# hanmekim/SceneLib2

Hardware: AMD Instinct MI355X
Metric: batched MonoSLAM frames/sec (320x240, 100 feat) (higher is better)
Workload: dtype f64

## Files before the change

scenelib2_amd/csrc/sl2_frontend.hip:

```cpp
#include "sl2_frontend_dev.hpp"

namespace sl2 {

__global__ void __launch_bounds__(256) k_predict(double* __restrict__ x, double* __restrict__ P, const int* __restrict__ n_slots,
                                                 double* __restrict__ prev_r, const int* __restrict__ part_i, int pend, int ld,
                                                 double* __restrict__ seq_time, const uint8_t* __restrict__ active) {
  if (!active[blockIdx.x]) { predict_paused(blockIdx.x, seq_time); return; }
  predict_body(blockIdx.x, x, P, n_slots, prev_r, part_i, pend, ld, seq_time);
}

__global__ void __launch_bounds__(64) k_feature_prediction(const double* __restrict__ x, const double* __restrict__ P,
                                                           const double* __restrict__ xp_org, int* __restrict__ f_flags,
                                                           const int* __restrict__ n_slots, double* __restrict__ f_h,
                                                           double* __restrict__ f_Hx, double* __restrict__ f_Hy,
                                                           double* __restrict__ f_R, double* __restrict__ f_S,
                                                           double* __restrict__ f_score, int* __restrict__ srch_i, double* __restrict__ srch_d,
                                                           const double* __restrict__ seq_cam, int width, int height, int N, int ld,
                                                           const uint8_t* __restrict__ active) {
  if (!active[blockIdx.y]) return;
  const CameraParams cam = load_cam(seq_cam, blockIdx.y, width, height);
  feature_prediction_body(blockIdx.y, blockIdx.x * blockDim.x + threadIdx.x, x, P, xp_org, f_flags, n_slots, f_h, f_Hx, f_Hy, f_R, f_S,
                          f_score, srch_i, srch_d, cam, N, ld);
}

__global__ void __launch_bounds__(256) k_select(const double* __restrict__ f_score, int* __restrict__ f_flags,
                                                const int* __restrict__ n_slots, const double* __restrict__ xp_org,
                                                int* __restrict__ sel_idx, int* __restrict__ n_sel, int* __restrict__ n_vis,
                                                double* __restrict__ last_r, const int* __restrict__ srch_i,
                                                const double* __restrict__ srch_d, int* __restrict__ srch_sel, int N,
                                                int n_want, int* __restrict__ srch_big, int split_bands,
                                                const uint8_t* __restrict__ active, int* __restrict__ sel_gate) {
  extern __shared__ double s_dyn[];
  if (!active[blockIdx.x]) { select_paused(blockIdx.x, sel_gate); return; }
  select_body(blockIdx.x, f_score, f_flags, n_slots, xp_org, sel_idx, n_sel, n_vis, last_r, srch_i, srch_d, srch_sel, N, n_want,
              srch_big, split_bands, s_dyn, sel_gate);
}

__global__ void __launch_bounds__(128) k_finalize(double* __restrict__ x, double* __restrict__ P, int* __restrict__ f_flags,
                                                  const int* __restrict__ n_slots, int* __restrict__ attempted,
                                                  int* __restrict__ successful, const int* __restrict__ m_count,
                                                  const int* __restrict__ n_sel, double* __restrict__ traj,
                                                  int* __restrict__ traj_count, const double* __restrict__ last_r,
                                                  int* __restrict__ status, double* __restrict__ pos_log, int* __restrict__ pos_count, int N, int ld,
                                                  int min_attempts, double match_fraction, int save_trajectory,
                                                  const int* __restrict__ part_i, int pend, int* __restrict__ slots_max,
                                                  unsigned long long* __restrict__ slots_mail, int publish,
                                                  const uint8_t* __restrict__ active, int* __restrict__ seq_age) {
  extern __shared__ int s_del[];
  if (!active[blockIdx.x]) { finalize_paused(blockIdx.x, x, n_slots, pos_log, pos_count, seq_age, ld, slots_max, slots_mail, publish); return; }
  finalize_body(blockIdx.x, x, P, f_flags, n_slots, attempted, successful, m_count, n_sel, traj, traj_count, last_r, status, pos_log,
                pos_count, N, ld, min_attempts, match_fraction, save_trajectory, part_i, pend, s_del, slots_max, slots_mail, publish);
}

#ifdef SL2_FRONT_TRACE
}
extern "C" int sl2_debug_front_trace(long long* dev_buf) {
  return hipMemcpyToSymbol(HIP_SYMBOL(sl2::g_front_trace), &dev_buf, sizeof(dev_buf)) == hipSuccess ? 0 : 2;
}
namespace sl2 {
#endif

int launch_predict(sl2_engine* e) {
  LaunchScope ls(e, "k_predict");
  hipLaunchKernelGGL(k_predict, dim3(e->B), dim3(256), 0, e->stream, e->x, e->P, e->n_slots, e->prev_r, e->part_i, e->ppos + 6 * e->kpart, e->ld,
                     e->seq_time, e->active);
  SL2_HIP(hipGetLastError());
  return SL2_OK;
}

int launch_feature_prediction(sl2_engine* e) {
  LaunchScope ls(e, "k_feature_prediction");
  dim3 grid((e->N + 63) / 64, e->B);
  hipLaunchKernelGGL(k_feature_prediction, grid, dim3(64), 0, e->stream, e->x, e->P, e->xp_org, e->f_flags, e->n_slots,
                     e->f_h, e->f_Hx, e->f_Hy, e->f_R, e->f_S, e->f_score, e->srch_i, e->srch_d, e->seq_cam, e->cam.width, e->cam.height, e->N, e->ld,
                     e->active);
  SL2_HIP(hipGetLastError());
  return SL2_OK;
}

int launch_select(sl2_engine* e, int n) {
  LaunchScope ls(e, "k_select");
  if (n > e->nsel_max) n = e->nsel_max;
  const size_t shm = (size_t)e->N * (sizeof(double) + 3 * sizeof(int));
  hipLaunchKernelGGL(k_select, dim3(e->B), dim3(256), shm, e->stream, e->f_score, e->f_flags, e->n_slots, e->xp_org,
                     e->sel_idx, e->n_sel, e->n_vis, e->last_r, e->srch_i, e->srch_d, e->srch_sel, e->N, n, e->srch_big,
                     (e->srch_big && e->root->search_variant == 1) ? e->root->search_split : 0, e->active, e->sel_gate);
  SL2_HIP(hipGetLastError());
  return SL2_OK;
}

int launch_finalize(sl2_engine* e, int save_trajectory) {
  LaunchScope ls(e, "k_finalize");
  const size_t shm = (size_t)e->N * 2 * sizeof(int);
  hipLaunchKernelGGL(k_finalize, dim3(e->B), dim3(128), shm, e->stream, e->x, e->P, e->f_flags, e->n_slots, e->attempted,
                     e->successful, e->m_count, e->n_sel, e->traj, e->traj_count, e->last_r, e->status, e->pos_log,
                     e->pos_count, e->N, e->ld, e->prm.minimum_attempted_measurements_of_feature,
                     e->prm.successful_match_fraction, save_trajectory, e->part_i, e->ppos + 6 * e->kpart, e->root->slots_max_dev,
                     e->root->slots_mail_dev, e->group_first == 0 ? 1 : 0, e->active, e->seq_age);
  SL2_HIP(hipGetLastError());
  return SL2_OK;
}

}
```

scenelib2_amd/csrc/sl2_frontend_dev.hpp:

```cpp
#pragma once
#include "sl2_common.hpp"

namespace sl2 {

#ifdef SL2_FRONT_TRACE
static __device__ long long* g_front_trace = nullptr;
#define FTR(kern, slot) do { if (g_front_trace && threadIdx.x == 0) g_front_trace[((size_t)(kern) * 4096 + blockIdx.x) * 8 + (slot)] = (long long)__builtin_readcyclecounter(); } while (0)
#else
#define FTR(kern, slot) do { } while (0)
#endif

__device__ __forceinline__ void predict_body(const int b, double* __restrict__ x, double* __restrict__ P, const int* __restrict__ n_slots,
                                                 double* __restrict__ prev_r, const int* __restrict__ part_i, int pend, int ld,
                                                 double* __restrict__ seq_time) {
  const int tid = threadIdx.x;
  double* xb = x + (size_t)b * ld;
  double* Pb = P + (size_t)b * ld * ld;
  FTR(0, 0);
  if (tid < 3) prev_r[b * 3 + tid] = xb[tid];
  const int n_used = part_i[(size_t)b * kPartInts + kPartCount] ? pend : 13 + 3 * n_slots[b];
  double v0[13];
  for (int k = 0; k < 13; ++k) v0[k] = (13 + tid < n_used) ? Pb[(size_t)k * ld + 13 + tid] : 0.0;
  __shared__ double s_f[13], s_A[16], s_B[12], s_P[169], s_T[169], s_dt;
  if (tid == 0) {
    double* rec = seq_time + (size_t)b * kSeqTimeDoubles;
    const double dt0 = rec[kSeqTimeNominal] + rec[kSeqTimeOwed];
    double xv[13];
    for (int i = 0; i < 13; ++i) xv[i] = xb[i];
    rec[kSeqTimeUsed] = dt0;
    rec[kSeqTimeOwed] = 0.0;
    s_dt = dt0;
    double f[13], A44[16], B43[12];
    motion_f_and_blocks(xv, dt0, f, A44, B43);
    for (int i = 0; i < 13; ++i) s_f[i] = f[i];
    for (int i = 0; i < 16; ++i) s_A[i] = A44[i];
    for (int i = 0; i < 12; ++i) s_B[i] = B43[i];
  }
  for (int e = tid; e < 169; e += blockDim.x) s_P[e] = Pb[(size_t)(e / 13) * ld + (e % 13)];
  __syncthreads();
  const double dt = s_dt;
  FTR(0, 1);
  for (int e = tid; e < 169; e += blockDim.x) {
    const int i = e / 13, j = e % 13;
    double v[13];
    for (int k = 0; k < 13; ++k) v[k] = s_P[k * 13 + j];
    s_T[e] = frow_dot(i, dt, s_A, s_B, v);
  }
  __syncthreads();
  FTR(0, 2);
  for (int e = tid; e < 169; e += blockDim.x) {
    const int i = e / 13, j = e % 13;
    double v[13];
    for (int k = 0; k < 13; ++k) v[k] = s_T[i * 13 + k];
    Pb[(size_t)i * ld + j] = frow_dot(j, dt, s_A, s_B, v) + process_noise_entry(i, j, dt, s_B);
  }
  FTR(0, 3);
  __shared__ double s_W[256][13];
  for (int j0 = 13; j0 < n_used; j0 += blockDim.x) {
    const int j = j0 + tid;
    if (j < n_used) {
      double v[13], w[13];
      for (int k = 0; k < 13; ++k) v[k] = (j0 == 13) ? v0[k] : Pb[(size_t)k * ld + j];
      for (int i = 0; i < 13; ++i) w[i] = frow_dot(i, dt, s_A, s_B, v);
      for (int i = 0; i < 13; ++i) {
        Pb[(size_t)i * ld + j] = w[i];
        s_W[tid][i] = w[i];
      }
    }
    __syncthreads();
    const int rr = tid >> 4, cc = tid & 15;
    for (int r0 = 0; r0 < (int)blockDim.x; r0 += blockDim.x / 16) {
      const int jr = j0 + r0 + rr;
      if (cc < 13 && jr < n_used) Pb[(size_t)jr * ld + cc] = s_W[r0 + rr][cc];
    }
    __syncthreads();
  }
  if (tid < 13) xb[tid] = s_f[tid];
  FTR(0, 4);
}

__device__ __forceinline__ void predict_paused(const int b, double* __restrict__ seq_time) {
  if (threadIdx.x == 0) {
    double* rec = seq_time + (size_t)b * kSeqTimeDoubles;
    if (rec[kSeqTimeCatchUp] != 0.0) rec[kSeqTimeOwed] += rec[kSeqTimeNominal];
  }
}

__device__ __forceinline__ void feature_prediction_body(const int b, const int i, const double* __restrict__ x, const double* __restrict__ P,
                                                           const double* __restrict__ xp_org, int* __restrict__ f_flags,
                                                           const int* __restrict__ n_slots, double* __restrict__ f_h,
                                                           double* __restrict__ f_Hx, double* __restrict__ f_Hy,
                                                           double* __restrict__ f_R, double* __restrict__ f_S,
                                                           double* __restrict__ f_score, int* __restrict__ srch_i, double* __restrict__ srch_d,
                                                           const CameraParams& cam, int N, int ld) {
  if (i >= n_slots[b]) return;
  const size_t fi = (size_t)b * N + i;
  int flags = f_flags[fi] & ~(FF_SELECTED | FF_VISIBLE);
  if (!(flags & FF_ACTIVE)) { f_flags[fi] = flags; return; }
  const double* xb = x + (size_t)b * ld;
  const double* Pb = P + (size_t)b * ld * ld;
  double xp[7], y[3], xo[7];
  for (int k = 0; k < 7; ++k) xp[k] = xb[k];
  const int pos = 13 + 3 * i;
  for (int k = 0; k < 3; ++k) y[k] = xb[pos + k];
  for (int k = 0; k < 7; ++k) xo[k] = xp_org[fi * 8 + k];
  double zeroed[3], h[2], Hx[14], Hy[6], Rn;
  measurement_model(cam, xp, y, zeroed, h, Hx, Hy, &Rn);
  double Pxx7[49], Pxy7[21], Pyy[9], S[4];
  for (int r = 0; r < 7; ++r) {
    for (int c = 0; c < 7; ++c) Pxx7[r * 7 + c] = Pb[(size_t)r * ld + c];
    for (int c = 0; c < 3; ++c) Pxy7[r * 3 + c] = Pb[(size_t)r * ld + pos + c];
  }
  for (int r = 0; r < 3; ++r)
    for (int c = 0; c < 3; ++c) Pyy[r * 3 + c] = Pb[(size_t)(pos + r) * ld + pos + c];
  innovation_cov(Hx, Hy, Rn, Pxx7, Pxy7, Pyy, S);
  const int cant_see = visibility_test(cam, xp, y, xo, h);
  f_h[fi * 2 + 0] = h[0]; f_h[fi * 2 + 1] = h[1];
  for (int k = 0; k < 14; ++k) f_Hx[fi * 14 + k] = Hx[k];
  for (int k = 0; k < 6; ++k) f_Hy[fi * 6 + k] = Hy[k];
  f_R[fi] = Rn;
  for (int k = 0; k < 4; ++k) f_S[fi * 4 + k] = S[k];
  f_score[fi] = S[0] + S[3];
  if (cant_see == 0) flags |= FF_VISIBLE;
  f_flags[fi] = flags;
  {
    double a, bq, c;
    sinv_from_S(S, &a, &bq, &c);
    const SearchBounds sb = search_bounds(h, a, bq, c, cam.width, cam.height);
    int* si = srch_i + fi * 8;
    si[0] = sb.ucentre; si[1] = sb.vcentre; si[2] = sb.urelstart; si[3] = sb.urelfinish - sb.urelstart + 1;
    si[4] = sb.vrelstart; si[5] = sb.vrelfinish - sb.vrelstart + 1; si[6] = sb.halfwidth; si[7] = sb.halfheight;
    double* sd = srch_d + fi * 4;
    sd[0] = a; sd[1] = bq; sd[2] = c; sd[3] = 0.0;
  }
}

__device__ __forceinline__ void select_body(const int b, const double* __restrict__ f_score, int* __restrict__ f_flags,
                                                const int* __restrict__ n_slots, const double* __restrict__ xp_org,
                                                int* __restrict__ sel_idx, int* __restrict__ n_sel, int* __restrict__ n_vis,
                                                double* __restrict__ last_r, const int* __restrict__ srch_i,
                                                const double* __restrict__ srch_d, int* __restrict__ srch_sel, int N,
                                                int n_want, int* __restrict__ srch_big, int split_bands, double* s_dyn,
                                                int* __restrict__ sel_gate) {
  double* s_score = s_dyn;
  int* s_vis = (int*)(s_dyn + N);
  int* s_nu = s_vis + N;
  __shared__ int s_nvis, s_zero_rank, s_last;
  const int tid = threadIdx.x;
  FTR(1, 0);
  const int ns = n_slots[b];
  if (tid == 0) { s_nvis = 0; s_zero_rank = 0x7fffffff; s_last = -1; }
  __syncthreads();
  for (int i0 = 0; i0 < ns; i0 += blockDim.x) {
    const int i = i0 + tid;
    int last = -1;
    if (i < ns) {
      const int fl = f_flags[(size_t)b * N + i];
      s_score[i] = f_score[(size_t)b * N + i];
      s_vis[i] = (fl & FF_VISIBLE) ? 1 : 0;
      if (fl & FF_ACTIVE) last = i;
    }
    for (int off = 32; off > 0; off >>= 1) last = max(last, __shfl_xor(last, off, 64));
    if ((tid & 63) == 0 && last >= 0) atomicMax(&s_last, last);
  }
  __syncthreads();
  FTR(1, 1);
  for (int i = tid; i < ns; i += blockDim.x) {
    if (!s_vis[i]) s_score[i] = -1.0;
    else if (s_score[i] != s_score[i]) s_score[i] = -0.5;
    s_nu[i] = 0;
  }
  __syncthreads();
  {
    const int G = (ns + 63) / 64 * 64;
    int P = G > 0 ? (int)blockDim.x / G : 1;
    P = P < 1 ? 1 : (P > 4 ? 4 : P);
    const int part = P > 1 ? tid / G : 0;
    for (int i = P > 1 ? tid - part * G : tid; i < ns && part < P; i += P > 1 ? ns : (int)blockDim.x) {
      if (!s_vis[i]) continue;
      const double si = s_score[i];
      const int j0 = part * ns / P, j1 = (part + 1) * ns / P;
      int rank = 0;
#pragma unroll 8
      for (int j = j0; j < j1; ++j) {
        const double sj = s_score[j];
        rank += (sj > si || (sj == si && j < i)) ? 1 : 0;
      }
      if (P > 1) atomicAdd(&s_nu[i], rank); else s_nu[i] = rank;
    }
  }
  __syncthreads();
  for (int i0 = 0; i0 < ns; i0 += blockDim.x) {
    const int i = i0 + tid;
    const bool vis = i < ns && s_vis[i];
    int zero_rank = 0x7fffffff;
    if (vis) {
      const int rank = s_nu[i];
      s_vis[i] = 1 + rank;
      if (s_score[i] == 0.0) zero_rank = rank;
    }
    const int nv = __popcll(__ballot(vis));
    for (int off = 32; off > 0; off >>= 1) zero_rank = min(zero_rank, __shfl_xor(zero_rank, off, 64));
    if ((tid & 63) == 0) {
      if (nv) atomicAdd(&s_nvis, nv);
      if (zero_rank != 0x7fffffff) atomicMin(&s_zero_rank, zero_rank);
    }
  }
  __syncthreads();
  FTR(1, 2);
  int limit = n_want;
  if (s_zero_rank < limit) limit = s_zero_rank;
  if (s_nvis < limit) limit = s_nvis;
  for (int i = tid; i < ns; i += blockDim.x) {
    if (!s_vis[i]) continue;
    const int rank = s_vis[i] - 1;
    if (rank < limit) {
      sel_idx[(size_t)b * N + rank] = i;
      f_flags[(size_t)b * N + i] |= FF_SELECTED;
      const int* si = srch_i + ((size_t)b * N + i) * 8;
      int* rec = srch_sel + ((size_t)b * N + rank) * 16;
      rec[0] = i;
#pragma unroll
      for (int q = 0; q < 7; ++q) rec[1 + q] = si[q];
      const double* sd = srch_d + ((size_t)b * N + i) * 4;
      double* recd = (double*)(rec + 8);
      recd[0] = sd[0]; recd[1] = sd[1]; recd[2] = sd[2];
      int shared = 0;
      if (split_bands > 0 && si[3] > 0 && si[5] > 0) {
        const int TU = (si[3] + 15) >> 4, TV = (si[5] + 15) >> 4;
        const int bands = ((TU + 1) >> 1) * TV;
        if (bands >= split_bands && TU <= 128 && TV <= 64) {
          const int per = srch_unit_bands(bands), units = (bands + per - 1) / per;
          const int u0 = atomicAdd(srch_big, units);
          if (u0 + units <= kSrchBigUnits) {
            int4 en;
            en.x = b; en.y = rank; en.z = u0; en.w = units;
            for (int q = 0; q < units; ++q) *(int4*)(srch_big + kSrchBigEntries + 4 * (u0 + q)) = en;
            atomicAdd(srch_big + 3, 1);
            shared = 1;
          } else {
            int4 en;
            en.x = -1; en.y = 0; en.z = 0; en.w = 0;
            for (int q = u0; q < min(u0 + units, kSrchBigUnits); ++q) *(int4*)(srch_big + kSrchBigEntries + 4 * q) = en;
          }
        }
      }
      rec[14] = shared ? si[3] : 0;
      if (shared) rec[4] = kSrchSharedNu;
    }
  }
  FTR(1, 3);
  if (tid == 0) {
    n_sel[b] = limit;
    sel_gate[b] = limit;
    n_vis[b] = s_nvis;
    if (s_last >= 0)
      for (int k = 0; k < 3; ++k) last_r[b * 3 + k] = xp_org[((size_t)b * N + s_last) * 8 + k];
  }
}

__device__ __forceinline__ void select_paused(const int b, int* __restrict__ sel_gate) {
  if (threadIdx.x == 0) sel_gate[b] = 0;
}
__device__ __forceinline__ void finalize_paused(const int b, const double* __restrict__ x, const int* __restrict__ n_slots,
                                                double* __restrict__ pos_log, int* __restrict__ pos_count, int* __restrict__ seq_age,
                                                int ld, int* __restrict__ slots_max, unsigned long long* __restrict__ slots_mail,
                                                int publish) {
  if (threadIdx.x != 0) return;
  const int pc = pos_count[b], ns = n_slots[b];
  pos_count[b] = pc + 1;
  seq_age[b] -= 1;
  const int log_slot = pc % kTrajCapacity;
  for (int k = 0; k < 3; ++k) pos_log[((size_t)b * kTrajCapacity + log_slot) * 3 + k] = x[(size_t)b * ld + k];
  if (slots_max) {
    if (ns > __hip_atomic_load(&slots_max[pc & 1], __ATOMIC_RELAXED, __HIP_MEMORY_SCOPE_AGENT)) atomicMax(&slots_max[pc & 1], ns);
    if (publish && b == 0) {
      const int prev = __hip_atomic_load(&slots_max[(pc + 1) & 1], __ATOMIC_RELAXED, __HIP_MEMORY_SCOPE_AGENT);
      __hip_atomic_store(&slots_max[(pc + 1) & 1], 0, __ATOMIC_RELAXED, __HIP_MEMORY_SCOPE_AGENT);
      __hip_atomic_store(slots_mail, ((unsigned long long)(unsigned)pc << 32) | (unsigned)prev, __ATOMIC_RELAXED, __HIP_MEMORY_SCOPE_SYSTEM);
    }
  }
}

template <bool kExtScratch = false>
__device__ __forceinline__ void finalize_body(const int b, double* __restrict__ x, double* __restrict__ P, int* __restrict__ f_flags,
                                                  const int* __restrict__ n_slots, int* __restrict__ attempted,
                                                  int* __restrict__ successful, const int* __restrict__ m_count,
                                                  const int* __restrict__ n_sel, double* __restrict__ traj,
                                                  int* __restrict__ traj_count, const double* __restrict__ last_r,
                                                  int* __restrict__ status, double* __restrict__ pos_log, int* __restrict__ pos_count, int N, int ld,
                                                  int min_attempts, double match_fraction, int save_trajectory,
                                                  const int* __restrict__ part_i, int pend, int* s_del,
                                              int* __restrict__ slots_max = nullptr, unsigned long long* __restrict__ slots_mail = nullptr,
                                              int publish = 0, double* s_ext = nullptr) {
  double *s_N, *s_P, *s_T;
  if constexpr (kExtScratch) {
    s_N = s_ext; s_P = s_ext + 16; s_T = s_ext + 16 + 169;
  } else {
    __shared__ double s_N_own[16], s_P_own[169], s_T_own[169];
    s_N = s_N_own; s_P = s_P_own; s_T = s_T_own;
  }
  __shared__ int s_ndel;
  const int tid = threadIdx.x;
  double* xb = x + (size_t)b * ld;
  double* Pb = P + (size_t)b * ld * ld;
  const int ns = n_slots[b];
  const int n_used = part_i[(size_t)b * kPartInts + kPartCount] ? pend : 13 + 3 * ns;
  const bool updated = (n_sel[b] > 0) && (m_count[b] > 0);
  constexpr int kStripCols = 6;
  double pre_P[2];
#pragma unroll
  for (int q = 0; q < 2; ++q) {
    const int e = tid + q * (int)blockDim.x;
    pre_P[q] = (e < 169) ? Pb[(size_t)(e / 13) * ld + (e % 13)] : 0.0;
  }
  const bool strip_in_regs = updated && (n_used - 13 <= kStripCols * (int)blockDim.x);
  double pre_v[kStripCols][4];
  if (strip_in_regs) {
#pragma unroll
    for (int q = 0; q < kStripCols; ++q) {
      const int j = 13 + tid + q * (int)blockDim.x;
#pragma unroll
      for (int k = 0; k < 4; ++k) pre_v[q][k] = (j < n_used) ? Pb[(size_t)(3 + k) * ld + j] : 0.0;
    }
  }
  int pre_fl = 0, pre_att = 0, pre_suc = 0;
  if (tid < ns) { const size_t fi = (size_t)b * N + tid; pre_fl = f_flags[fi]; pre_att = attempted[fi]; pre_suc = successful[fi]; }
  double pre_x[13], pre_lr[3];
  int pre_tc = 0, pre_pc = 0;
  if (tid == 0) {
    for (int k = 0; k < 13; ++k) pre_x[k] = xb[k];
    for (int k = 0; k < 3; ++k) pre_lr[k] = last_r[b * 3 + k];
    pre_tc = traj_count[b]; pre_pc = pos_count[b];
  }
#pragma unroll
  for (int q = 0; q < 2; ++q) {
    const int e = tid + q * (int)blockDim.x;
    if (e < 169) s_P[e] = pre_P[q];
  }
  if (updated) {
    if (tid == 0) {
      double q[4] = {pre_x[3], pre_x[4], pre_x[5], pre_x[6]}, Nn[16];
      dqnorm_by_dq(q, Nn);
      for (int i = 0; i < 16; ++i) s_N[i] = Nn[i];
    }
    __syncthreads();
    for (int e = tid; e < 169; e += blockDim.x) {
      const int i = e / 13, j = e % 13;
      double v;
      if (i >= 3 && i < 7) {
        v = 0.0;
        for (int k = 0; k < 4; ++k) v += s_N[(i - 3) * 4 + k] * s_P[(3 + k) * 13 + j];
      } else v = s_P[e];
      s_T[e] = v;
    }
    __syncthreads();
    for (int e = tid; e < 169; e += blockDim.x) {
      const int i = e / 13, j = e % 13;
      double v;
      if (j >= 3 && j < 7) {
        v = 0.0;
        for (int k = 0; k < 4; ++k) v += s_T[i * 13 + 3 + k] * s_N[(j - 3) * 4 + k];
      } else v = s_T[e];
      s_P[e] = v;
    }
    if (strip_in_regs) {
#pragma unroll
      for (int q = 0; q < kStripCols; ++q) {
        const int j = 13 + tid + q * (int)blockDim.x;
        if (j < n_used) {
          double w[4];
          for (int a = 0; a < 4; ++a) {
            double acc = 0.0;
            for (int k = 0; k < 4; ++k) acc += s_N[a * 4 + k] * pre_v[q][k];
            w[a] = acc;
          }
          for (int a = 0; a < 4; ++a) {
            Pb[(size_t)(3 + a) * ld + j] = w[a];
            Pb[(size_t)j * ld + 3 + a] = w[a];
          }
        }
      }
    } else {
      for (int j = 13 + tid; j < n_used; j += blockDim.x) {
        double v[4], w[4];
        for (int k = 0; k < 4; ++k) v[k] = Pb[(size_t)(3 + k) * ld + j];
        for (int a = 0; a < 4; ++a) {
          double acc = 0.0;
          for (int k = 0; k < 4; ++k) acc += s_N[a * 4 + k] * v[k];
          w[a] = acc;
        }
        for (int a = 0; a < 4; ++a) {
          Pb[(size_t)(3 + a) * ld + j] = w[a];
          Pb[(size_t)j * ld + 3 + a] = w[a];
        }
      }
    }
    __syncthreads();
  } else {
    __syncthreads();
  }
  for (int i = tid; i < ns; i += blockDim.x) {
    const size_t fi = (size_t)b * N + i;
    const bool first = i == tid;
    int fl = first ? pre_fl : f_flags[fi];
    if (fl & FF_ACTIVE) {
      const int att = first ? pre_att : attempted[fi], suc = first ? pre_suc : successful[fi];
      if (att >= min_attempts && double(suc) / double(att) < match_fraction) { fl |= FF_SCHEDULED; f_flags[fi] = fl; }
    }
    s_del[N + i] = fl;
  }
  __syncthreads();
  if (tid == 0) s_ndel = 0;
  __syncthreads();
  for (int i = tid; i < ns; i += blockDim.x) {
    const int fl = s_del[N + i];
    if ((fl & FF_ACTIVE) && (fl & FF_SCHEDULED)) {
      int run = 0;
      for (int j = i - 1; j >= 0; --j) {
        const int fj = s_del[N + j];
        if (fj & FF_PARTIAL) break;
        if (!(fj & FF_ACTIVE)) continue;
        if (!(fj & FF_SCHEDULED)) break;
        ++run;
      }
      if ((run & 1) == 0) {
        f_flags[(size_t)b * N + i] = FF_USED;
        s_del[atomicAdd(&s_ndel, 1)] = i;
      }
    }
  }
  __syncthreads();
  for (int d = 0; d < s_ndel; ++d) {
    const int pos = 13 + 3 * s_del[d];
    for (int j = tid; j < n_used; j += blockDim.x)
      for (int r = 0; r < 3; ++r) {
        Pb[(size_t)(pos + r) * ld + j] = 0.0;
        Pb[(size_t)j * ld + pos + r] = 0.0;
      }
  }
  for (int e = tid; e < 169; e += blockDim.x) {
    const int i = e / 13, j = e % 13;
    Pb[(size_t)i * ld + j] = s_P[i * 13 + j] * 0.5 + s_P[j * 13 + i] * 0.5;
  }
  if (tid == 0) {
    if (save_trajectory) {
      const int c = pre_tc;
      double* t = traj + ((size_t)b * kTrajCapacity + (c % kTrajCapacity)) * 3;
      for (int k = 0; k < 3; ++k) t[k] = pre_lr[k];
      traj_count[b] = c + 1;
    }
    const int log_slot = pre_pc % kTrajCapacity;
    pos_count[b] = pre_pc + 1;
    for (int k = 0; k < 3; ++k) pos_log[((size_t)b * kTrajCapacity + log_slot) * 3 + k] = pre_x[k];
    bool bad = false;
    for (int k = 0; k < 13; ++k) bad = bad || !isfinite(pre_x[k]) || !isfinite(s_P[k * 13 + k]);
    if (bad) status[b] |= 1;
    if (slots_max) {
      if (ns > __hip_atomic_load(&slots_max[pre_pc & 1], __ATOMIC_RELAXED, __HIP_MEMORY_SCOPE_AGENT)) atomicMax(&slots_max[pre_pc & 1], ns);
      if (publish && b == 0) {
        const int prev = __hip_atomic_load(&slots_max[(pre_pc + 1) & 1], __ATOMIC_RELAXED, __HIP_MEMORY_SCOPE_AGENT);
        __hip_atomic_store(&slots_max[(pre_pc + 1) & 1], 0, __ATOMIC_RELAXED, __HIP_MEMORY_SCOPE_AGENT);
        __hip_atomic_store(slots_mail, ((unsigned long long)(unsigned)pre_pc << 32) | (unsigned)prev, __ATOMIC_RELAXED, __HIP_MEMORY_SCOPE_SYSTEM);
      }
    }
  }
}


}
```

Measured before the change: 1.032 million.

## Specialize predict kernel waves and stage Pxx via lane broadcast in feature prediction

The predict kernel is restructured so three waves prefetch and transform covariance strip columns in registers while a fourth wave computes the motion model, process noise and the 13x13 block using only wave-level syncs. Block-wide barriers and serial phases in the predict step are meant to shrink, with transposed writes staged through shared memory. Feature prediction now loads the shared 7x7 pose covariance once per wave and broadcasts it with readlane instead of each thread issuing 49 global loads. Wave-level tracing hooks are also added under a debug macro. The cost is extra register pressure and a hard-coded 3+1 wave split.

Measured after the change: 1.009 million. 0.978x the previous value.

```diff
diff --git a/scenelib2_amd/csrc/sl2_frontend.hip b/scenelib2_amd/csrc/sl2_frontend.hip
--- a/scenelib2_amd/csrc/sl2_frontend.hip
+++ b/scenelib2_amd/csrc/sl2_frontend.hip
@@ -6,7 +6,7 @@
                                                  double* __restrict__ prev_r, const int* __restrict__ part_i, int pend, int ld,
                                                  double* __restrict__ seq_time, const uint8_t* __restrict__ active) {
   if (!active[blockIdx.x]) { predict_paused(blockIdx.x, seq_time); return; }
-  predict_body(blockIdx.x, x, P, n_slots, prev_r, part_i, pend, ld, seq_time);
+  predict_body_waves(blockIdx.x, x, P, n_slots, prev_r, part_i, pend, ld, seq_time);
 }
 
 __global__ void __launch_bounds__(64) k_feature_prediction(const double* __restrict__ x, const double* __restrict__ P,
@@ -19,8 +19,8 @@
                                                            const uint8_t* __restrict__ active) {
   if (!active[blockIdx.y]) return;
   const CameraParams cam = load_cam(seq_cam, blockIdx.y, width, height);
-  feature_prediction_body(blockIdx.y, blockIdx.x * blockDim.x + threadIdx.x, x, P, xp_org, f_flags, n_slots, f_h, f_Hx, f_Hy, f_R, f_S,
-                          f_score, srch_i, srch_d, cam, N, ld);
+  feature_prediction_body<true>(blockIdx.y, blockIdx.x * blockDim.x + threadIdx.x, x, P, xp_org, f_flags, n_slots, f_h, f_Hx, f_Hy, f_R, f_S,
+                                f_score, srch_i, srch_d, cam, N, ld);
 }
 
 __global__ void __launch_bounds__(256) k_select(const double* __restrict__ f_score, int* __restrict__ f_flags,
@@ -56,6 +56,9 @@
 }
 extern "C" int sl2_debug_front_trace(long long* dev_buf) {
   return hipMemcpyToSymbol(HIP_SYMBOL(sl2::g_front_trace), &dev_buf, sizeof(dev_buf)) == hipSuccess ? 0 : 2;
+}
+extern "C" int sl2_debug_front_wave_trace(long long* dev_buf) {
+  return hipMemcpyToSymbol(HIP_SYMBOL(sl2::g_front_wtrace), &dev_buf, sizeof(dev_buf)) == hipSuccess ? 0 : 2;
 }
 namespace sl2 {
 #endif
diff --git a/scenelib2_amd/csrc/sl2_frontend_dev.hpp b/scenelib2_amd/csrc/sl2_frontend_dev.hpp
--- a/scenelib2_amd/csrc/sl2_frontend_dev.hpp
+++ b/scenelib2_amd/csrc/sl2_frontend_dev.hpp
@@ -6,9 +6,21 @@
 #ifdef SL2_FRONT_TRACE
 static __device__ long long* g_front_trace = nullptr;
 #define FTR(kern, slot) do { if (g_front_trace && threadIdx.x == 0) g_front_trace[((size_t)(kern) * 4096 + blockIdx.x) * 8 + (slot)] = (long long)__builtin_readcyclecounter(); } while (0)
+static __device__ long long* g_front_wtrace = nullptr;
+#define FTW(kern, wg, slot) do { if (g_front_wtrace && (threadIdx.x & 63) == 0) g_front_wtrace[(((size_t)(kern) * 4096 + (wg)) * 4 + (threadIdx.x >> 6)) * 8 + (slot)] = (long long)__builtin_readcyclecounter(); } while (0)
 #else
 #define FTR(kern, slot) do { } while (0)
+#define FTW(kern, wg, slot) do { } while (0)
 #endif
+
+__device__ __forceinline__ double bcast_lane_f64(double v, int lane) {
+  return __hiloint2double(__builtin_amdgcn_readlane(__double2hiint(v), lane), __builtin_amdgcn_readlane(__double2loint(v), lane));
+}
+__device__ __forceinline__ void wave_lds_sync() {
+  __builtin_amdgcn_fence(__ATOMIC_RELEASE, "wavefront");
+  __builtin_amdgcn_wave_barrier();
+  __builtin_amdgcn_fence(__ATOMIC_ACQUIRE, "wavefront");
+}
 
 __device__ __forceinline__ void predict_body(const int b, double* __restrict__ x, double* __restrict__ P, const int* __restrict__ n_slots,
                                                  double* __restrict__ prev_r, const int* __restrict__ part_i, int pend, int ld,
@@ -79,6 +91,136 @@
   FTR(0, 4);
 }
 
+constexpr int kPredictStripThreads = 192, kPredictPreCols = 2 * kPredictStripThreads;
+__device__ __forceinline__ void predict_body_waves(const int b, double* __restrict__ x, double* __restrict__ P, const int* __restrict__ n_slots,
+                                                   double* __restrict__ prev_r, const int* __restrict__ part_i, int pend, int ld,
+                                                   double* __restrict__ seq_time) {
+  const int tid = threadIdx.x;
+  const bool strip_wave = tid < kPredictStripThreads;
+  double* xb = x + (size_t)b * ld;
+  double* Pb = P + (size_t)b * ld * ld;
+  FTW(0, b, 0);
+  __shared__ double s_f[13], s_A[16], s_B[12], s_P[169], s_T[169], s_dt;
+  __shared__ double s_W[kPredictPreCols][7];
+  const int n_used = part_i[(size_t)b * kPartInts + kPartCount] ? pend : 13 + 3 * n_slots[b];
+  double v[2][13], prev = 0.0;
+  if (strip_wave) {
+#pragma unroll
+    for (int q = 0; q < 2; ++q) {
+      const int j = 13 + tid + q * kPredictStripThreads;
+#pragma unroll
+      for (int k = 0; k < 13; ++k) v[q][k] = (j < n_used) ? Pb[(size_t)k * ld + j] : 0.0;
+    }
+    if (tid < 3) prev = xb[tid];
+  } else {
+    const int l = tid - kPredictStripThreads;
+    double xv[13], pxx[3], qn[3];
+    double* rec = seq_time + (size_t)b * kSeqTimeDoubles;
+    for (int i = 0; i < 13; ++i) xv[i] = xb[i];
+    const double dt0 = rec[kSeqTimeNominal] + rec[kSeqTimeOwed];
+#pragma unroll
+    for (int q = 0; q < 3; ++q) {
+      const int e = l + 64 * q;
+      pxx[q] = (e < 169) ? Pb[(size_t)(e / 13) * ld + (e % 13)] : 0.0;
+    }
+    if (l == 0) {
+      rec[kSeqTimeUsed] = dt0;
+      rec[kSeqTimeOwed] = 0.0;
+      s_dt = dt0;
+      double f[13], A44[16], B43[12];
+      motion_f_and_blocks(xv, dt0, f, A44, B43);
+      for (int i = 0; i < 13; ++i) s_f[i] = f[i];
+      for (int i = 0; i < 16; ++i) s_A[i] = A44[i];
+      for (int i = 0; i < 12; ++i) s_B[i] = B43[i];
+    }
+    wave_lds_sync();
+#pragma unroll
+    for (int q = 0; q < 3; ++q) {
+      const int e = l + 64 * q;
+      qn[q] = (e < 169) ? process_noise_entry(e / 13, e % 13, dt0, s_B) : 0.0;
+    }
+#pragma unroll
+    for (int q = 0; q < 3; ++q) {
+      const int e = l + 64 * q;
+      if (e < 169) s_P[e] = pxx[q];
+    }
+    wave_lds_sync();
+#pragma unroll
+    for (int q = 0; q < 3; ++q) {
+      const int e = l + 64 * q;
+      if (e < 169) {
+        const int i = e / 13, j = e % 13;
+        double u[13];
+        for (int k = 0; k < 13; ++k) u[k] = s_P[k * 13 + j];
+        s_T[e] = frow_dot(i, dt0, s_A, s_B, u);
+      }
+    }
+    wave_lds_sync();
+    FTW(0, b, 1);
+#pragma unroll
+    for (int q = 0; q < 3; ++q) {
+      const int e = l + 64 * q;
+      if (e < 169) {
+        const int i = e / 13, j = e % 13;
+        double u[13];
+        for (int k = 0; k < 13; ++k) u[k] = s_T[i * 13 + k];
+        Pb[(size_t)i * ld + j] = frow_dot(j, dt0, s_A, s_B, u) + qn[q];
+      }
+    }
+    FTW(0, b, 2);
+  }
+  if (strip_wave) { FTW(0, b, 1); FTW(0, b, 2); }
+  __syncthreads();
+  const double dt = s_dt;
+  FTW(0, b, 3);
+  if (strip_wave) {
+    if (tid < 3) prev_r[b * 3 + tid] = prev;
+#pragma unroll
+    for (int q = 0; q < 2; ++q) {
+      const int c = tid + q * kPredictStripThreads, j = 13 + c;
+      if (j < n_used) {
+        double w[7];
+#pragma unroll
+        for (int i = 0; i < 7; ++i) w[i] = frow_dot(i, dt, s_A, s_B, v[q]);
+#pragma unroll
+        for (int i = 0; i < 7; ++i) {
+          Pb[(size_t)i * ld + j] = w[i];
+          s_W[c][i] = w[i];
+        }
+      }
+    }
+  }
+  FTW(0, b, 4);
+  __syncthreads();
+  FTW(0, b, 5);
+  {
+    const int rr = tid >> 3, cc = tid & 7;
+    const int n_pre = min(n_used - 13, kPredictPreCols);
+    for (int c = rr; c < n_pre; c += 32)
+      if (cc < 7) Pb[(size_t)(13 + c) * ld + cc] = s_W[c][cc];
+  }
+  FTW(0, b, 6);
+  for (int j0 = 13 + kPredictPreCols; j0 < n_used; j0 += 256) {
+    __syncthreads();
+    const int j = j0 + tid;
+    if (j < n_used) {
+      double u[13], w[7];
+      for (int k = 0; k < 13; ++k) u[k] = Pb[(size_t)k * ld + j];
+      for (int i = 0; i < 7; ++i) w[i] = frow_dot(i, dt, s_A, s_B, u);
+      for (int i = 0; i < 7; ++i) {
+        Pb[(size_t)i * ld + j] = w[i];
+        s_W[tid][i] = w[i];
+      }
+    }
+    __syncthreads();
+    const int rr = tid >> 3, cc = tid & 7;
+    for (int c = rr; c < 256 && j0 + c < n_used; c += 32)
+      if (cc < 7) Pb[(size_t)(j0 + c) * ld + cc] = s_W[c][cc];
+  }
+  if (tid < 13) xb[tid] = s_f[tid];
+  FTW(0, b, 7);
+}
+
 __device__ __forceinline__ void predict_paused(const int b, double* __restrict__ seq_time) {
   if (threadIdx.x == 0) {
     double* rec = seq_time + (size_t)b * kSeqTimeDoubles;
@@ -86,6 +228,7 @@
   }
 }
 
+template <bool kStaged = false>
 __device__ __forceinline__ void feature_prediction_body(const int b, const int i, const double* __restrict__ x, const double* __restrict__ P,
                                                            const double* __restrict__ xp_org, int* __restrict__ f_flags,
                                                            const int* __restrict__ n_slots, double* __restrict__ f_h,
@@ -93,28 +236,62 @@
                                                            double* __restrict__ f_R, double* __restrict__ f_S,
                                                            double* __restrict__ f_score, int* __restrict__ srch_i, double* __restrict__ srch_d,
                                                            const CameraParams& cam, int N, int ld) {
-  if (i >= n_slots[b]) return;
-  const size_t fi = (size_t)b * N + i;
-  int flags = f_flags[fi] & ~(FF_SELECTED | FF_VISIBLE);
-  if (!(flags & FF_ACTIVE)) { f_flags[fi] = flags; return; }
+#ifdef SL2_FRONT_TRACE
+  const int wg = blockIdx.y * gridDim.x + blockIdx.x;
+#endif
+  FTW(1, wg, 0);
   const double* xb = x + (size_t)b * ld;
   const double* Pb = P + (size_t)b * ld * ld;
+  const int pos = 13 + 3 * i;
+  const size_t fi = (size_t)b * N + i;
+  double Pxx7_own[49], Pxy7[21], Pyy[9], S[4];
   double xp[7], y[3], xo[7];
-  for (int k = 0; k < 7; ++k) xp[k] = xb[k];
-  const int pos = 13 + 3 * i;
-  for (int k = 0; k < 3; ++k) y[k] = xb[pos + k];
-  for (int k = 0; k < 7; ++k) xo[k] = xp_org[fi * 8 + k];
+  int flags = 0;
+  if constexpr (kStaged) {
+    const int l = threadIdx.x;
+    for (int k = 0; k < 7; ++k) xp[k] = xb[k];
+    const int ns = n_slots[b];
+    if (i - l >= ns) return;
+    const bool mine = i < ns;
+    const int ic = mine ? i : ns - 1, posc = 13 + 3 * ic;
+    const size_t fic = (size_t)b * N + ic;
+    flags = f_flags[fic];
+    for (int k = 0; k < 3; ++k) y[k] = xb[posc + k];
+    for (int k = 0; k < 7; ++k) xo[k] = xp_org[fic * 8 + k];
+    const double pv = (l < 49) ? Pb[(size_t)(l / 7) * ld + (l % 7)] : 0.0;
+    for (int r = 0; r < 7; ++r)
+      for (int c = 0; c < 3; ++c) Pxy7[r * 3 + c] = Pb[(size_t)r * ld + posc + c];
+    for (int r = 0; r < 3; ++r)
+      for (int c = 0; c < 3; ++c) Pyy[r * 3 + c] = Pb[(size_t)(posc + r) * ld + posc + c];
+    for (int k = 0; k < 49; ++k) Pxx7_own[k] = bcast_lane_f64(pv, k);
+    if (!mine) return;
+  } else {
+    if (i >= n_slots[b]) return;
+    flags = f_flags[fi];
+  }
+  flags &= ~(FF_SELECTED | FF_VISIBLE);
+  if (!(flags & FF_ACTIVE)) { f_flags[fi] = flags; return; }
+  if constexpr (!kStaged) {
+    for (int k = 0; k < 7; ++k) xp[k] = xb[k];
+    for (int k = 0; k < 3; ++k) y[k] = xb[pos + k];
+    for (int k = 0; k < 7; ++k) xo[k] = xp_org[fi * 8 + k];
+  }
   double zeroed[3], h[2], Hx[14], Hy[6], Rn;
   measurement_model(cam, xp, y, zeroed, h, Hx, Hy, &Rn);
-  double Pxx7[49], Pxy7[21], Pyy[9], S[4];
-  for (int r = 0; r < 7; ++r) {
-    for (int c = 0; c < 7; ++c) Pxx7[r * 7 + c] = Pb[(size_t)r * ld + c];
-    for (int c = 0; c < 3; ++c) Pxy7[r * 3 + c] = Pb[(size_t)r * ld + pos + c];
-  }
-  for (int r = 0; r < 3; ++r)
-    for (int c = 0; c < 3; ++c) Pyy[r * 3 + c] = Pb[(size_t)(pos + r) * ld + pos + c];
+  FTW(1, wg, 1);
+  const double* Pxx7 = Pxx7_own;
+  if constexpr (!kStaged) {
+    for (int r = 0; r < 7; ++r) {
+      for (int c = 0; c < 7; ++c) Pxx7_own[r * 7 + c] = Pb[(size_t)r * ld + c];
+      for (int c = 0; c < 3; ++c) Pxy7[r * 3 + c] = Pb[(size_t)r * ld + pos + c];
+    }
+    for (int r = 0; r < 3; ++r)
+      for (int c = 0; c < 3; ++c) Pyy[r * 3 + c] = Pb[(size_t)(pos + r) * ld + pos + c];
+  }
   innovation_cov(Hx, Hy, Rn, Pxx7, Pxy7, Pyy, S);
+  FTW(1, wg, 2);
   const int cant_see = visibility_test(cam, xp, y, xo, h);
+  FTW(1, wg, 3);
   f_h[fi * 2 + 0] = h[0]; f_h[fi * 2 + 1] = h[1];
   for (int k = 0; k < 14; ++k) f_Hx[fi * 14 + k] = Hx[k];
   for (int k = 0; k < 6; ++k) f_Hy[fi * 6 + k] = Hy[k];
@@ -133,6 +310,7 @@
     double* sd = srch_d + fi * 4;
     sd[0] = a; sd[1] = bq; sd[2] = c; sd[3] = 0.0;
   }
+  FTW(1, wg, 4);
 }
 
 __device__ __forceinline__ void select_body(const int b, const double* __restrict__ f_score, int* __restrict__ f_flags,
@@ -304,6 +482,7 @@
   const int tid = threadIdx.x;
   double* xb = x + (size_t)b * ld;
   double* Pb = P + (size_t)b * ld * ld;
+  FTW(2, b, 0);
   const int ns = n_slots[b];
   const int n_used = part_i[(size_t)b * kPartInts + kPartCount] ? pend : 13 + 3 * ns;
   const bool updated = (n_sel[b] > 0) && (m_count[b] > 0);
@@ -345,6 +524,7 @@
       for (int i = 0; i < 16; ++i) s_N[i] = Nn[i];
     }
     __syncthreads();
+    FTW(2, b, 1);
     for (int e = tid; e < 169; e += blockDim.x) {
       const int i = e / 13, j = e % 13;
       double v;
@@ -355,6 +535,7 @@
       s_T[e] = v;
     }
     __syncthreads();
+    FTW(2, b, 2);
     for (int e = tid; e < 169; e += blockDim.x) {
       const int i = e / 13, j = e % 13;
       double v;
@@ -400,6 +581,7 @@
   } else {
     __syncthreads();
   }
+  FTW(2, b, 3);
   for (int i = tid; i < ns; i += blockDim.x) {
     const size_t fi = (size_t)b * N + i;
     const bool first = i == tid;
@@ -411,6 +593,7 @@
     s_del[N + i] = fl;
   }
   __syncthreads();
+  FTW(2, b, 4);
   if (tid == 0) s_ndel = 0;
   __syncthreads();
   for (int i = tid; i < ns; i += blockDim.x) {
@@ -431,6 +614,7 @@
     }
   }
   __syncthreads();
+  FTW(2, b, 5);
   for (int d = 0; d < s_ndel; ++d) {
     const int pos = 13 + 3 * s_del[d];
     for (int j = tid; j < n_used; j += blockDim.x)
@@ -443,6 +627,7 @@
     const int i = e / 13, j = e % 13;
     Pb[(size_t)i * ld + j] = s_P[i * 13 + j] * 0.5 + s_P[j * 13 + i] * 0.5;
   }
+  FTW(2, b, 6);
   if (tid == 0) {
     if (save_trajectory) {
       const int c = pre_tc;
@@ -465,7 +650,8 @@
       }
     }
   }
-}
-
-
-}
+  FTW(2, b, 7);
+}
+
+
+}
```
